# paulmillr/noble-curves

Hardware: AMD Instinct MI355X
Metric: secp256k1_scalar_mults_per_sec (higher is better)
Workload: dtype u32

## Files before the change

### noble-curves_amd/csrc/ec_sw.hpp

```cpp
#pragma once
#include "fp2.hpp"

namespace ncg {

template <class A, class B, class C, class D>
NCG_DI auto f_mulsub(const A& a, const B& b, const C& c, const D& d) -> decltype(a * b - c * d) {
  return a * b - c * d;
}


template <class F>
struct Affine {
  F x, y;
  NCG_DI bool is_inf() const { return x.is_zero() && y.is_zero(); }
};

template <class F>
struct Jac {
  F X, Y, Z;
  static NCG_DI Jac inf() { return {F::one(), F::one(), F::zero()}; }
  NCG_DI bool is_inf() const { return Z.is_zero(); }
};

template <class F>
// ... 43 lines not shown
  auto S2 = qy * p.Z * Z1Z1;
  auto H = U2 - p.X;
  auto R = S2 - p.Y;
  if (f_eqz(H)) {
    if (f_eqz(R)) return jac_dbl(p);
    return Jac<F>::inf();
  }
  auto HH = f_sqr(H);
  auto HHH = H * HH;
  auto V = p.X * HH;
  auto X3 = f_sqr(R) - HHH - f_dbl(V);
  auto Y3 = R * (V - X3) - p.Y * HHH;
  auto Z3 = p.Z * H;
  return {X3, Y3, Z3};
}
template <class F, class FX, class FY>
NCG_DI Jac<F> jac_madd_q(const Jac<F>& p, const FX& qx, const FY& qy) {
  if (qx.is_zero() && qy.is_zero()) return p;
  if (p.is_inf()) return {qx, qy, F::one()};
  return jac_madd_xy(p, qx, qy);
}
template <class F>
NCG_DI Jac<F> jac_madd(const Jac<F>& p, const Affine<F>& q) {
  return jac_madd_q(p, q.x, q.y);
}

template <class F>
NCG_DI Jac<F> jac_add(const Jac<F>& p, const Jac<F>& q) {
  if (q.is_inf()) return p;
  if (p.is_inf()) return q;
  auto Z1Z1 = f_sqr(p.Z);
  auto Z2Z2 = f_sqr(q.Z);
  auto U1 = p.X * Z2Z2;
  auto U2 = q.X * Z1Z1;
  auto S1 = p.Y * q.Z * Z2Z2;
  auto S2 = q.Y * p.Z * Z1Z1;
  auto H = U2 - U1;
  auto R = S2 - S1;
  if (f_eqz(H)) {
    if (f_eqz(R)) return jac_dbl(p);
    return Jac<F>::inf();
  }
  auto HH = f_sqr(H);
  auto HHH = H * HH;
  auto V = U1 * HH;
  auto X3 = f_sqr(R) - HHH - f_dbl(V);
  auto Y3 = R * (V - X3) - S1 * HHH;
  auto Z3 = p.Z * q.Z * H;
  return {X3, Y3, Z3};
}

template <class F, class ZI>
NCG_DI Affine<F> jac_to_affine(const Jac<F>& p, const ZI& zinv) {
  if (p.is_inf()) return {F::zero(), F::zero()};
  auto zi2 = f_sqr(zinv);
  return {p.X * zi2, p.Y * zi2 * zinv};
}

template <class PR, int B>
NCG_DI Jac<Fe9<PR, B>> jac_dbl(const Jac<Fe9<PR, B>>& p) {
  auto A = f_sqr(p.X);
  auto Bq = f_sqr(p.Y);
  auto C8 = f_dbl(f_sqr(f_dbl(Bq)));
  auto D = fe9_norm(f_dbl(f_dbl(p.X * Bq)));
  auto E = fe9_norm(A + A + A);
  auto X3 = f_sqr(E) - f_dbl(D);
  auto Y3 = E * (D - X3) - C8;
  auto Z3 = f_dbl(p.Y * p.Z);
  return {X3, Y3, Z3};
}

template <class PR, int B, int BX, int BY>
NCG_DI Jac<Fe9<PR, B>> jac_madd_xy(const Jac<Fe9<PR, B>>& p, const Fe9<PR, BX>& qx, const Fe9<PR, BY>& qy) {
  using F = Fe9<PR, B>;
  auto Z1Z1 = f_sqr(p.Z);
  auto U2 = qx * Z1Z1;
  auto S2 = qy * (p.Z * Z1Z1);
  auto Hw = U2 - p.X;
  auto Rw = S2 - p.Y;
  if (f_eqz(Hw)) {
    if (f_eqz(Rw)) return jac_dbl(p);
    return Jac<F>::inf();
  }
  auto H = fe9_norm(Hw);
  auto R = fe9_norm(Rw);
  auto HH = f_sqr(H);
  auto HHH = H * HH;
  auto V = p.X * HH;
  auto X3 = fe9_norm(f_sqr(R) - HHH - f_dbl(V));
  auto Y3 = R * (V - X3) - p.Y * HHH;
  auto Z3 = p.Z * H;
  return {X3, Y3, Z3};
}
template <class PR, int B>
NCG_DI Jac<Fe9<PR, B>> jac_add(const Jac<Fe9<PR, B>>& p, const Jac<Fe9<PR, B>>& q) {
  using F = Fe9<PR, B>;
  if (q.is_inf()) return p;
  if (p.is_inf()) return q;
  auto Z1Z1 = f_sqr(p.Z);
  auto Z2Z2 = f_sqr(q.Z);
  auto U1 = p.X * Z2Z2;
  auto U2 = q.X * Z1Z1;
  auto S1 = p.Y * (q.Z * Z2Z2);
  auto S2 = q.Y * (p.Z * Z1Z1);
  auto Hw = U2 - U1;
  auto Rw = S2 - S1;
  if (f_eqz(Hw)) {
    if (f_eqz(Rw)) return jac_dbl(p);
    return Jac<F>::inf();
  }
  auto H = fe9_norm(Hw);
  auto R = fe9_norm(Rw);
  auto HH = f_sqr(H);
  auto HHH = H * HH;
  auto V = U1 * HH;
  auto X3 = fe9_norm(f_sqr(R) - HHH - f_dbl(V));
  auto Y3 = R * (V - X3) - S1 * HHH;
  auto Z3 = (p.Z * q.Z) * H;
  return {X3, Y3, Z3};
}

template <class PR, int B>
NCG_DI Jac<Fe9<PR, B>> jac_dbl_neg(const Jac<Fe9<PR, B>>& p) {
  auto A = f_sqr(p.X);
  auto S = f_sqr(p.Y);
  auto T = p.X * S;
  auto L = f_half(fe9_norm(A + A + A));
  auto X3 = f_sqr_add(L, f_neg_lin2(T));
  auto W = f_mul_sqr(L, X3 - T, S);
  auto Z3 = p.Y * p.Z;
  return {X3, W, Z3};
}

template <class PR, int B, int BX, int BY>
NCG_DI Jac<Fe9<PR, B>> jac_madd_neg(const Jac<Fe9<PR, B>>& p, const Fe9<PR, BX>& qx, const Fe9<PR, BY>& qy) {
  using F = Fe9<PR, B>;
  if (qx.is_zero() && qy.is_zero()) return {p.X, f_neg(p.Y), p.Z};
  if (p.is_inf()) return {qx, f_neg(qy), F::one()};
  auto Z1Z1 = f_sqr(p.Z);
  auto Z1Z1Z1 = p.Z * Z1Z1;
  auto H = f_mul_add(qx, Z1Z1, f_neg_lin(p.X));
  auto R = f_mul_add(qy, Z1Z1Z1, f_neg_lin(p.Y));
  if (f_eqz(H)) {
    if (f_eqz(R)) return jac_dbl_neg(p);
    return Jac<F>::inf();
  }
  auto HH = f_sqr(H);
  auto HHH = H * HH;
  auto V = p.X * HH;
  auto X3 = f_sqr_add(R, f_neg_lin(HHH, V));
  auto W = f_mul_mul(R, X3 - V, p.Y, HHH);
  auto Z3 = p.Z * H;
  return {X3, W, Z3};
}

template <class F>
NCG_DI Xyzz<F> xyzz_from_affine(const Affine<F>& p) {
  if (p.is_inf()) return Xyzz<F>::inf();
  return {p.x, p.y, F::one(), F::one()};
}

template <class F>
NCG_DI Xyzz<F> xyzz_mdbl(const Affine<F>& p) {
  auto U = f_dbl(p.y);
  auto V = f_sqr(U);
  auto W = U * V;
  auto S = p.x * V;
  auto xx = f_sqr(p.x);
  auto M = f_dbl(xx) + xx;
  auto X3 = f_sqr(M) - f_dbl(S);
  auto Y3 = f_mulsub(M, S - X3, W, p.y);
  return {X3, Y3, V, W};
}

template <class F>
NCG_DI Xyzz<F> xyzz_dbl(const Xyzz<F>& p) {
  if (p.is_inf()) return p;
  auto U = f_dbl(p.Y);
  auto V = f_sqr(U);
  auto W = U * V;
  auto S = p.X * V;
  auto xx = f_sqr(p.X);
  auto M = f_dbl(xx) + xx;
  auto X3 = f_sqr(M) - f_dbl(S);
  auto Y3 = f_mulsub(M, S - X3, W, p.Y);
  return {X3, Y3, V * p.ZZ, W * p.ZZZ};
}

template <class F>
NCG_DI Xyzz<F> xyzz_madd(const Xyzz<F>& p, const Affine<F>& q_in, bool neg = false) {
  if (q_in.is_inf()) return p;
  Affine<F> q = q_in;
  if (neg) q.y = f_neg(q.y);
  if (p.is_inf()) return {q.x, q.y, F::one(), F::one()};
  auto U2 = q.x * p.ZZ;
  auto S2 = q.y * p.ZZZ;
  auto Pq = U2 - p.X;
  auto R = S2 - p.Y;
  if (f_eqz(Pq)) {
    if (f_eqz(R)) return xyzz_mdbl(q);
    return Xyzz<F>::inf();
  }
  auto PP = f_sqr(Pq);
  auto PPP = Pq * PP;
  auto Q = p.X * PP;
  auto X3 = f_sqr(R) - PPP - f_dbl(Q);
  auto Y3 = f_mulsub(R, Q - X3, p.Y, PPP);
  return {X3, Y3, p.ZZ * PP, p.ZZZ * PPP};
}

template <class F>
NCG_DI Xyzz<F> xyzz_add(const Xyzz<F>& p, const Xyzz<F>& q) {
  if (q.is_inf()) return p;
  if (p.is_inf()) return q;
  auto U1 = p.X * q.ZZ;
  auto U2 = q.X * p.ZZ;
  auto S1 = p.Y * q.ZZZ;
  auto S2 = q.Y * p.ZZZ;
  auto Pq = U2 - U1;
  auto R = S2 - S1;
  if (f_eqz(Pq)) {
    if (f_eqz(R)) return xyzz_dbl(p);
    return Xyzz<F>::inf();
  }
  auto PP = f_sqr(Pq);
  auto PPP = Pq * PP;
  auto Q = U1 * PP;
  auto X3 = f_sqr(R) - PPP - f_dbl(Q);
  auto Y3 = f_mulsub(R, Q - X3, S1, PPP);
  return {X3, Y3, p.ZZ * q.ZZ * PP, p.ZZZ * q.ZZZ * PPP};
}

template <class PR, int B>
NCG_DI Xyzz<Fe9<PR, B>> xyzz_mdbl(const Affine<Fe9<PR, B>>& p) {
  auto U = f_dbl(p.y);
  auto V = f_sqr(U);
  auto W = U * V;
  auto S = p.x * V;
  auto xx = f_sqr(p.x);
  auto M = fe9_norm(xx + xx + xx);
  auto X3 = fe9_norm(f_sqr(M) - f_dbl(S));
  auto Y3 = M * (S - X3) - W * p.y;
  return {X3, Y3, V, W};
}
template <class PR, int B>
NCG_DI Xyzz<Fe9<PR, B>> xyzz_dbl(const Xyzz<Fe9<PR, B>>& p) {
  if (p.is_inf()) return p;
  auto U = f_dbl(p.Y);
  auto V = f_sqr(U);
  auto W = U * V;
  auto S = p.X * V;
  auto xx = f_sqr(p.X);
  auto M = fe9_norm(xx + xx + xx);
  auto X3 = fe9_norm(f_sqr(M) - f_dbl(S));
  auto Y3 = M * (S - X3) - W * p.Y;
  return {X3, Y3, V * p.ZZ, W * p.ZZZ};
}
template <class PR, int B>
NCG_DI Xyzz<Fe9<PR, B>> xyzz_madd(const Xyzz<Fe9<PR, B>>& p, const Affine<Fe9<PR, B>>& q_in, bool neg = false) {
  using F = Fe9<PR, B>;
  if (q_in.is_inf()) return p;
  const Fe9<PR, B + 1> qy = neg ? f_neg(q_in.y) : Fe9<PR, B + 1>(q_in.y);
  if (p.is_inf()) return {q_in.x, qy, F::one(), F::one()};
  auto U2 = q_in.x * p.ZZ;
  auto S2 = qy * p.ZZZ;
  auto Pw = U2 - p.X;
  auto Rw = S2 - p.Y;
  if (f_eqz(Pw)) {
    if (f_eqz(Rw)) return xyzz_mdbl(Affine<F>{q_in.x, qy});
    return Xyzz<F>::inf();
  }
  auto Pq = fe9_norm(Pw);
  auto R = fe9_norm(Rw);
  auto PP = f_sqr(Pq);
  auto PPP = Pq * PP;
  auto Q = p.X * PP;
  auto X3 = fe9_norm(f_sqr(R) - PPP - f_dbl(Q));
  auto Y3 = R * (Q - X3) - p.Y * PPP;
  return {X3, Y3, p.ZZ * PP, p.ZZZ * PPP};
}
template <class PR, int B>
NCG_DI Xyzz<Fe9<PR, B>> xyzz_add(const Xyzz<Fe9<PR, B>>& p, const Xyzz<Fe9<PR, B>>& q) {
  using F = Fe9<PR, B>;
  if (q.is_inf()) return p;
  if (p.is_inf()) return q;
  auto U1 = p.X * q.ZZ;
  auto U2 = q.X * p.ZZ;
  auto S1 = p.Y * q.ZZZ;
  auto S2 = q.Y * p.ZZZ;
  auto Pw = U2 - U1;
  auto Rw = S2 - S1;
  if (f_eqz(Pw)) {
    if (f_eqz(Rw)) return xyzz_dbl(p);
    return Xyzz<F>::inf();
  }
  auto Pq = fe9_norm(Pw);
  auto R = fe9_norm(Rw);
  auto PP = f_sqr(Pq);
  auto PPP = Pq * PP;
  auto Q = U1 * PP;
  auto X3 = fe9_norm(f_sqr(R) - PPP - f_dbl(Q));
  auto Y3 = R * (Q - X3) - S1 * PPP;
  return {X3, Y3, (p.ZZ * q.ZZ) * PP, (p.ZZZ * q.ZZZ) * PPP};
}

}
// ... 1 lines not shown
```

### noble-curves_amd/csrc/fe9.hpp

```cpp
#pragma once
#include <type_traits>

#include "fp.hpp"
#include "fe9_asm_gen.hpp"
#include "fe9m.hpp"

namespace ncg {

constexpr uint32_t FE9_MASK = (1u << 29) - 1u;

template <class PR, class = void> struct Fe9IsMont : std::false_type {};
template <class PR> struct Fe9IsMont<PR, std::void_t<decltype(PR::MONT)>> : std::integral_constant<bool, PR::MONT> {};

template <class PR>
struct Fe9Raw {
  uint32_t v[9];
};

NCG_DI void fe9_mac(uint64_t& acc, uint32_t a, uint32_t b) {
#ifdef __HIP_DEVICE_COMPILE__
  asm("v_mad_u64_u32 %0, vcc, %1, %2, %0" : "+v"(acc) : "v"(a), "v"(b) : "vcc");
#else
  acc += (uint64_t)a * b;
#endif
// ... 224 lines not shown
  static NCG_DI Fe9 zero() {
    Fe9 r;
#pragma unroll
    for (int i = 0; i < 9; i++) r.v[i] = 0;
    return r;
  }
  static NCG_DI Fe9 one() {
    Fe9 r = zero();
    if constexpr (Fe9IsMont<PR>::value) {
#pragma unroll
      for (int i = 0; i < 9; i++) r.v[i] = PR::ONE[i];
    } else {
      r.v[0] = 1;
    }
    return r;
  }
  template <class ARR>
  static NCG_DI Fe9 from_limbs(const ARR& a) {
    Fe9 r;
#pragma unroll
    for (int i = 0; i < 9; i++) r.v[i] = a[i];
    return r;
  }
  NCG_DI bool is_zero() const {
    uint32_t o = 0;
#pragma unroll
    for (int i = 0; i < 9; i++) o |= v[i];
    return o == 0;
  }
};

template <class PR, int B>
NCG_DI Fe9<PR, 1> fe9_norm(const Fe9<PR, B>& a) {
  if constexpr (B == 1) return a;
  else return Fe9<PR, 1>(a);
}

template <class PR, int A, int B>
NCG_DI Fe9<PR, A + B> operator+(const Fe9<PR, A>& a, const Fe9<PR, B>& b) {
  Fe9<PR, A + B> r;
#pragma unroll
  for (int i = 0; i < 9; i++) r.v[i] = a.v[i] + b.v[i];
  return r;
}
template <class PR, int A, int B>
NCG_DI Fe9<PR, A + B + 1> operator-(const Fe9<PR, A>& a, const Fe9<PR, B>& b) {
  Fe9<PR, A + B + 1> r;
#pragma unroll
  for (int i = 0; i < 9; i++) {
#ifdef __HIP_DEVICE_COMPILE__
    asm("v_sad_u32 %0, %1, %2, %3" : "=v"(r.v[i]) : "s"(PR::BIAS[B][i]), "v"(b.v[i]), "v"(a.v[i]));
#else
    r.v[i] = a.v[i] + (PR::BIAS[B][i] - b.v[i]);
#endif
  }
  return r;
}
template <class PR, int A>
NCG_DI Fe9<PR, A + 1> f_neg(const Fe9<PR, A>& a) {
  Fe9<PR, A + 1> r;
  const bool z = a.is_zero();
#pragma unroll
  for (int i = 0; i < 9; i++) r.v[i] = z ? 0u : PR::BIAS[A][i] - a.v[i];
  return r;
}
template <class PR, int A>
NCG_DI Fe9<PR, 2 * A> f_dbl(const Fe9<PR, A>& a) {
  Fe9<PR, 2 * A> r;
#pragma unroll
  for (int i = 0; i < 9; i++) r.v[i] = a.v[i] << 1;
  return r;
}

template <class PR, int A, int B>
NCG_DI Fe9<PR, 1> operator*(const Fe9<PR, A>& a, const Fe9<PR, B>& b) {
  if constexpr (A * B > 7) {
    if constexpr (A >= B) return fe9_norm(a) * b;
    else return a * fe9_norm(b);
  } else {
    Fe9Raw<PR> x, y;
#pragma unroll
    for (int i = 0; i < 9; i++) {
      x.v[i] = a.v[i];
      y.v[i] = b.v[i];
    }
    const Fe9Raw<PR> z = fe9_mul_raw<PR>(x, y);
    Fe9<PR, 1> r;
#pragma unroll
    for (int i = 0; i < 9; i++) r.v[i] = z.v[i];
    return r;
  }
}
template <class PR, int A>
NCG_DI Fe9<PR, 1> f_sqr(const Fe9<PR, A>& a) {
  if constexpr (A > 2) {
    return f_sqr(fe9_norm(a));
  } else {
    Fe9Raw<PR> x;
#pragma unroll
    for (int i = 0; i < 9; i++) x.v[i] = a.v[i];
    const Fe9Raw<PR> z = fe9_sqr_raw<PR>(x);
    Fe9<PR, 1> r;
#pragma unroll
    for (int i = 0; i < 9; i++) r.v[i] = z.v[i];
    return r;
  }
}

template <class PR, int KIND, int A, int B, int C, int D>
NCG_DI Fe9<PR, 1> fe9_fused(const Fe9<PR, A>& a, const Fe9<PR, B>& b, const Fe9<PR, C>& f, const Fe9<PR, D>& g) {
  Fe9<PR, 1> r;
  fe9_fused_limbs<PR, KIND>(r.v, a.v, b.v, f.v, g.v);
  return r;
}
template <class PR, int A, int B, int C, int D>
NCG_DI Fe9<PR, 1> f_mul_mul(const Fe9<PR, A>& a, const Fe9<PR, B>& b, const Fe9<PR, C>& c, const Fe9<PR, D>& d) {
  static_assert(A * B + C * D <= 7, "fused a*b + c*d: the two products overflow the 64-bit columns");
  return fe9_fused<PR, FE9_MM>(a, b, c, d);
}
template <class PR, int A, int B, int C>
NCG_DI Fe9<PR, 1> f_mul_sqr(const Fe9<PR, A>& a, const Fe9<PR, B>& b, const Fe9<PR, C>& c) {
  static_assert(C <= 2 && A * B + C * C <= 7, "fused a*b + c^2: the two sources overflow the 64-bit columns");
  return fe9_fused<PR, FE9_MS>(a, b, c, f_dbl(c));
}
template <class PR, int A, int B, int S>
NCG_DI Fe9<PR, 1> f_mul_add(const Fe9<PR, A>& a, const Fe9<PR, B>& b, const Fe9<PR, S>& s) {
  static_assert(A * B <= 7, "fused a*b + s: the product overflows the 64-bit columns");
  return fe9_fused<PR, FE9_MA>(a, b, s, s);
}
template <class PR, int A, int S>
NCG_DI Fe9<PR, 1> f_sqr_add(const Fe9<PR, A>& a, const Fe9<PR, S>& s) {
  static_assert(A <= 2, "fused a^2 + s: the square overflows the 64-bit columns");
  return fe9_fused<PR, FE9_SA>(a, f_dbl(a), s, s);
}
template <class PR, int S1, int S2>
NCG_DI Fe9<PR, S1 + 2 * S2 + 1> f_neg_lin(const Fe9<PR, S1>& s1, const Fe9<PR, S2>& s2) {
  Fe9<PR, S1 + 2 * S2 + 1> r;
#pragma unroll
  for (int i = 0; i < 9; i++) r.v[i] = PR::BIAS[S1 + 2 * S2][i] - (s1.v[i] + (s2.v[i] << 1));
  return r;
}
template <class PR, int S1>
NCG_DI Fe9<PR, S1 + 1> f_neg_lin(const Fe9<PR, S1>& s1) {
  Fe9<PR, S1 + 1> r;
#pragma unroll
  for (int i = 0; i < 9; i++) r.v[i] = PR::BIAS[S1][i] - s1.v[i];
  return r;
}
template <class PR, int S2>
NCG_DI Fe9<PR, 2 * S2 + 1> f_neg_lin2(const Fe9<PR, S2>& s2) {
  Fe9<PR, 2 * S2 + 1> r;
#pragma unroll
  for (int i = 0; i < 9; i++) r.v[i] = PR::BIAS[2 * S2][i] - (s2.v[i] << 1);
  return r;
}
template <class PR>
NCG_DI Fe9<PR, 2> f_half(const Fe9<PR, 1>& a) {
  const uint32_t m = 0u - (a.v[0] & 1u);
  uint32_t t[9];
#pragma unroll
  for (int i = 0; i < 9; i++) t[i] = a.v[i] + (PR::P[i] & m);
  Fe9<PR, 2> r;
#pragma unroll
  for (int i = 0; i < 8; i++) r.v[i] = (t[i] >> 1) + ((t[i + 1] & 1u) << 28);
  r.v[8] = t[8] >> 1;
  return r;
}

template <class PR>
NCG_DI Fe9<PR, 1> fe9_sqr_n(Fe9<PR, 1> a, int n) {
  for (int i = 0; i < n; i++) a = f_sqr(a);
  return a;
}

template <class PR, int A>
NCG_DI void fe9_canon_limbs_sf(uint32_t (&o)[9], const Fe9<PR, A>& a);
template <class PR, int A>
NCG_DI void fe9_canon_limbs(uint32_t (&o)[9], const Fe9<PR, A>& a) {
  if constexpr (Fe9IsMont<PR>::value) {
    uint32_t t[9];
    fe9m_reduce(t, a.v);
    fe9m_cond_sub(o, t);
  } else {
    fe9_canon_limbs_sf<PR, A>(o, a);
  }
}
template <class PR, int A>
NCG_DI void fe9_canon_limbs_sf(uint32_t (&o)[9], const Fe9<PR, A>& a) {
  uint64_t cy = 0;
  uint32_t t[9];
#pragma unroll
  for (int i = 0; i < 9; i++) {
    cy += a.v[i];
    t[i] = (uint32_t)cy & FE9_MASK;
    cy >>= 29;
  }
#pragma unroll
  for (int pass = 0; pass < 2; pass++) {
    uint64_t e = (uint64_t)(uint32_t)cy * PR::C0 + t[0];
    t[0] = (uint32_t)e & FE9_MASK;
    e >>= 29;
    e += (uint64_t)(uint32_t)cy * PR::C1 + t[1];
    t[1] = (uint32_t)e & FE9_MASK;
    e >>= 29;
#pragma unroll
    for (int i = 2; i < 9; i++) {
      e += t[i];
      t[i] = (uint32_t)e & FE9_MASK;
      e >>= 29;
    }
    cy = e;
  }
  constexpr int PBITS = (PR::P[8] >> 23) ? 256 : 255;
  constexpr int TOPB = PBITS - 232;
  constexpr uint32_t CSM = (uint32_t)((1ull << 29) - PR::P[0]);
  constexpr uint32_t CS1 = FE9_MASK - PR::P[1];
#pragma unroll
  for (int pass = 0; pass < 2; pass++) {
    const uint32_t q = t[8] >> TOPB;
    t[8] &= (1u << TOPB) - 1u;
    uint64_t e = (uint64_t)q * CSM + t[0];
    t[0] = (uint32_t)e & FE9_MASK;
    e >>= 29;
    e += (uint64_t)q * CS1 + t[1];
    t[1] = (uint32_t)e & FE9_MASK;
    e >>= 29;
#pragma unroll
    for (int i = 2; i < 9; i++) {
      e += t[i];
      t[i] = (uint32_t)e & FE9_MASK;
      e >>= 29;
    }
  }
  uint32_t s[9];
  int32_t bw = 0;
#pragma unroll
  for (int i = 0; i < 9; i++) {
    int32_t dd = (int32_t)t[i] - (int32_t)PR::P[i] + bw;
    s[i] = (uint32_t)dd & FE9_MASK;
    bw = dd >> 29;
  }
  const bool ge = bw == 0;
#pragma unroll
  for (int i = 0; i < 9; i++) o[i] = ge ? s[i] : t[i];
}

template <class PR, class... T>
__host__ __device__ __noinline__ bool fe9_eqz_slow(T... limbs) {
  Fe9<PR, 7> a;
  const uint32_t v[9] = {limbs...};
#pragma unroll
  for (int i = 0; i < 9; i++) a.v[i] = v[i];
  uint32_t c[9];
  fe9_canon_limbs<PR, 7>(c, a);
  uint32_t o = 0;
#pragma unroll
  for (int i = 0; i < 9; i++) o |= c[i];
  return o == 0;
}
template <class PR, int A>
NCG_DI bool f_eqz(const Fe9<PR, A>& a) {
  const uint32_t j = (a.v[0] * PR::PINV) & FE9_MASK;
  if (j >= (uint32_t)(PR::JMAX * A)) return false;
  return fe9_eqz_slow<PR>(a.v[0], a.v[1], a.v[2], a.v[3], a.v[4], a.v[5], a.v[6], a.v[7], a.v[8]);
}
template <class PR, int A, int B>
NCG_DI bool f_eq(const Fe9<PR, A>& a, const Fe9<PR, B>& b) {
  return f_eqz(a - b);
}

template <class PR>
NCG_DI Fe9<PR, 1> fe9_from_wire(const uint32_t* __restrict__ p) {
  if constexpr (Fe9IsMont<PR>::value) {
    Fe9<PR, 1> r;
    fe9m_from_wire(r.v, p);
    return r;
  }
  uint32_t w[10];
#pragma unroll
  for (int i = 0; i < 8; i++) w[i] = p[i];
  w[8] = 0;
  w[9] = 0;
  Fe9<PR, 1> r;
#pragma unroll
  for (int i = 0; i < 9; i++) {
    const int bit = 29 * i, limb = bit >> 5, sh = bit & 31;
    const uint64_t two = ((uint64_t)w[limb + 1] << 32) | w[limb];
    r.v[i] = (uint32_t)(two >> sh) & FE9_MASK;
  }
  return r;
}
template <class PR, int A>
NCG_DI void fe9_to_wire(uint32_t* __restrict__ p, const Fe9<PR, A>& a) {
  if constexpr (Fe9IsMont<PR>::value) {
    uint32_t c[9];
    fe9m_canon_plain(c, fe9_norm(a).v);
    fe9m_words_from_limbs(p, c);
    return;
  }
  uint32_t l[11];
  uint32_t c[9];
  fe9_canon_limbs<PR, A>(c, a);
#pragma unroll
  for (int i = 0; i < 9; i++) l[i] = c[i];
  l[9] = 0;
  l[10] = 0;
// ... 77 lines not shown
```

### noble-curves_amd/csrc/hosttest.hip

```cpp
#include <vector>

#include "../../include/ncg.h"
#include "mulvar.hpp"
#include "ed25519.hip"
#include "decode.hip"
#include "ntt.hip"
#include "poly.hip"
#include "h2c.hip"
#include "endo.hpp"
#include "ecdsa.hip"
#include "msm_shard.hpp"
#include "msm_endo.hip"
#include "msm_schedule.hpp"
#include "fe9m_check.hpp"
#include "group_check.hpp"
#include "x25519.hip"
#include "ristretto.hip"

using namespace ncg;

template <class C, int W>
static void ht_mul_var_t(const uint32_t* pts, const uint32_t* scalars, uint32_t* out, uint8_t* out_inf, int n) {
  constexpr int FW = MulVarCfg<C, W>::FW, WW = MulVarCfg<C, W>::WW;
  std::vector<uint32_t> tab(MulVarCfg<C, W>::TS * 2 * FW);
// ... 192 lines not shown
  }
  Fe9<PR, 1> o;
  if constexpr (A * B + C * D <= 7) {
    if (op == 0) o = f_mul_mul(x, y, z, w);
  }
  if constexpr (C <= 2 && A * B + C * C <= 7) {
    if (op == 1) o = f_mul_sqr(x, y, z);
  }
  if constexpr (A * B <= 7) {
    if (op == 2) o = f_mul_add(x, y, z);
  }
  if constexpr (A <= 2) {
    if (op == 3) o = f_sqr_add(x, z);
  }
  if constexpr (A == 1) {
    if (op == 4) {
      const Fe9<PR, 2> h = f_half(x);
      for (int i = 0; i < 9; i++) r[i] = h.v[i];
      return;
    }
  }
  for (int i = 0; i < 9; i++) r[i] = o.v[i];
}
template <class PR>
static int ht_fe9_fused_t(int op, int variant, const uint32_t* a, const uint32_t* b, const uint32_t* c, const uint32_t* d, uint32_t* r) {
  switch (variant) {
    case 1111: ht_fe9_fused_ab<PR, 1, 1, 1, 1>(op, a, b, c, d, r); return 0;
    case 1322: ht_fe9_fused_ab<PR, 1, 3, 2, 2>(op, a, b, c, d, r); return 0;
    case 3211: ht_fe9_fused_ab<PR, 3, 2, 1, 1>(op, a, b, c, d, r); return 0;
    case 2311: ht_fe9_fused_ab<PR, 2, 3, 1, 1>(op, a, b, c, d, r); return 0;
    case 1123: ht_fe9_fused_ab<PR, 1, 1, 2, 3>(op, a, b, c, d, r); return 0;
    case 3121: ht_fe9_fused_ab<PR, 3, 1, 2, 1>(op, a, b, c, d, r); return 0;
    case 1327: ht_fe9_fused_ab<PR, 1, 3, 2, 7>(op, a, b, c, d, r); return 0;
    case 7171: ht_fe9_fused_ab<PR, 7, 1, 7, 1>(op, a, b, c, d, r); return 0;
    case 1771: ht_fe9_fused_ab<PR, 1, 7, 7, 1>(op, a, b, c, d, r); return 0;
    case 2171: ht_fe9_fused_ab<PR, 2, 1, 7, 1>(op, a, b, c, d, r); return 0;
    default: return -1;
  }
}

template <class F>
static int fr29_op_host(int op, const uint32_t* a, const uint32_t* b, uint32_t* r) {
  Fr29 x, y, z;
  for (int i = 0; i < 9; i++) {
    x.v[i] = a[i];
    y.v[i] = b ? b[i] : 0;
    z.v[i] = 0;
  }
  fr29_overflows() = 0;
  switch (op) {
    case 0: z = fr29_mont<F>(x, y); break;
    case 1: z = fr29_add(x, y); break;
    case 2: z = fr29_sub<F>(x, y); break;
    case 3: z = fr29_weak(x); break;
    case 4: z = fr29_reduce256<F>(x); break;
    case 5: z = fr29_cond_sub<F>(x); break;
    case 8: z = fr29_fold255<F>(x); break;
    case 6: {
      uint32_t w[8];
      for (int i = 0; i < 8; i++) w[i] = a[i];
      z = fr29_from_words(w);
      break;
    }
    case 7: {
      uint32_t w[8];
      fr29_to_words(w, x);
      for (int i = 0; i < 8; i++) z.v[i] = w[i];
      z.v[8] = 0;
      break;
    }
    default: return -1;
  }
  for (int i = 0; i < 9; i++) r[i] = z.v[i];
  return fr29_overflows();
}

template <class PR, int A>
static void ht_fe9_inv_batch_t(int which, const uint32_t* a, uint32_t* out, uint32_t* raw, int n) {
  for (int k = 0; k < n; k++) {
    Fe9<PR, A> x;
    for (int i = 0; i < 9; i++) x.v[i] = a[(size_t)k * 9 + i];
    const Fe9<PR, 1> z = which ? f_inv_fermat(x) : f_inv(x);
    fe9_to_wire(out + (size_t)k * 8, z);
    if (raw)
      for (int i = 0; i < 9; i++) raw[(size_t)k * 9 + i] = z.v[i];
  }
}

extern "C" {

int ht_fe9_op(int field, int op, int variant, const uint32_t* a, const uint32_t* b, uint32_t* r) {
  if (field == 0) return ht_fe9_t<Fe9SecpPR>(op, variant, a, b, r);
  if (field == 1) return ht_fe9_t<Fe9EdPR>(op, variant, a, b, r);
  return -1;
}

int ht_fe9_inv_batch(int field, int A, int which, const uint32_t* a, uint32_t* out, uint32_t* raw, int n) {
  if (field < 0 || field > 1 || (A != 1 && A != 2 && A != 7)) return -1;
#define CALL(PR) (A == 1 ? ht_fe9_inv_batch_t<PR, 1>(which, a, out, raw, n) : A == 2 ? ht_fe9_inv_batch_t<PR, 2>(which, a, out, raw, n) : ht_fe9_inv_batch_t<PR, 7>(which, a, out, raw, n))
  if (field == 0) CALL(Fe9SecpPR);
  else CALL(Fe9EdPR);
#undef CALL
  return 0;
}

int ht_mul_var(int curve, const uint32_t* pts, const uint32_t* scalars, uint32_t* out, uint8_t* out_inf, int n) {
  switch (curve) {
    case CURVE_SECP256K1: ht_mul_var_t<CurveSecp, 4>(pts, scalars, out, out_inf, n); return 0;
    case CURVE_BLS12_381_G1: ht_mul_var_t<CurveG1, 3>(pts, scalars, out, out_inf, n); return 0;
    case 12: ht_mul_var_t<CurveG1E, 4>(pts, scalars, out, out_inf, n); return 0;
    case 14: ht_mul_var_t<CurveSecpI, 4>(pts, scalars, out, out_inf, n); return 0;
    case CURVE_BLS12_381_G2: ht_mul_var_t<CurveG2, 3>(pts, scalars, out, out_inf, n); return 0;
    case CURVE_BN254_G1: ht_mul_var_t<CurveBn254, 4>(pts, scalars, out, out_inf, n); return 0;
  }
  return -1;
}

int ht_field_op(int field, int op, const uint32_t* a, const uint32_t* b, uint32_t* r) {
  switch (field) {
    case 0: ht_field_t<ParamsSecpP>(op, a, b, r); return 0;
    case 1: ht_field_t<ParamsEdP>(op, a, b, r); return 0;
    case 2: ht_field_t<ParamsBlsP>(op, a, b, r); return 0;
  }
  return -1;
}

int ht_fe9_fused(int field, int op, int variant, const uint32_t* a, const uint32_t* b, const uint32_t* c, const uint32_t* d,
                 uint32_t* r) {
  if (field == 0) return ht_fe9_fused_t<Fe9SecpPR>(op, variant, a, b, c, d, r);
  if (field == 1) return ht_fe9_fused_t<Fe9EdPR>(op, variant, a, b, c, d, r);
  return -1;
}

int ht_jac_neg(int op, const uint32_t* p, const uint32_t* qx, const uint32_t* qy, uint32_t* out) {
  Jac<FeSecp> P;
  Fe9<Fe9SecpPR, 2> x;
  Fe9<Fe9SecpPR, 3> y;
  for (int i = 0; i < 9; i++) {
    P.X.v[i] = p[i];
    P.Y.v[i] = p[9 + i];
    P.Z.v[i] = p[18 + i];
    x.v[i] = qx[i];
    y.v[i] = qy[i];
  }
  Jac<FeSecp> R;
  if (op == 0) R = jac_dbl_neg(P);
  else if (op == 1) R = jac_madd_neg(P, x, y);
  else return -1;
  for (int i = 0; i < 9; i++) {
    out[i] = R.X.v[i];
    out[9 + i] = R.Y.v[i];
    out[18 + i] = R.Z.v[i];
  }
  return 0;
}

int ht_glv_split_odd(const uint32_t* k, uint32_t* out) {
  uint32_t kk[8];
  for (int i = 0; i < 8; i++) kk[i] = k[i];
  GlvSplit s = secp_glv_split(kk);
  secp_glv_make_odd(s);
  for (int i = 0; i < 5; i++) {
    out[i] = s.k1[i];
    out[5 + i] = s.k2[i];
  }
  out[10] = s.k1neg;
  out[11] = s.k2neg;
  return 0;
}

int ht_glv_split_k1_odd(const uint32_t* k, uint32_t* out) {
  uint32_t kk[8];
  for (int i = 0; i < 8; i++) kk[i] = k[i];
  GlvSplit s = secp_glv_split(kk);
  secp_glv_make_k1_odd(s);
  for (int i = 0; i < 5; i++) {
    out[i] = s.k1[i];
    out[5 + i] = s.k2[i];
  }
  out[10] = s.k1neg;
  out[11] = s.k2neg;
  return 0;
}

int ht_glv_split(const uint32_t* k, uint32_t* out) {
  uint32_t kk[8];
  for (int i = 0; i < 8; i++) kk[i] = k[i];
  GlvSplit s = secp_glv_split(kk);
  for (int i = 0; i < 5; i++) {
    out[i] = s.k1[i];
    out[5 + i] = s.k2[i];
  }
  out[10] = s.k1neg;
  out[11] = s.k2neg;
  return 0;
}

int ht_ed25519_mul_var(const uint32_t* pts, const uint32_t* scalars, uint32_t* out, uint8_t* out_inf, int n) {
  for (int i = 0; i < n; i++) ed25519_mul_var_host(pts + (size_t)i * 16, scalars + (size_t)i * 8, out + (size_t)i * 16, out_inf + i);
  return 0;
}

int ht_x25519(const uint32_t* scalars, const uint32_t* u, int flags, uint32_t* out, uint8_t* ok, int n) {
  if (flags & ~1) return -1;
  x25519_host(scalars, u, flags & 1, out, ok, n);
  return 0;
}
int ht_x25519_base(const uint32_t* scalars, uint32_t* out, uint8_t* ok, int n) {
  x25519_base_host(scalars, out, ok, n);
  return 0;
}
int ht_ed25519_to_montgomery(const uint32_t* pk, uint32_t* out, uint8_t* ok, int n) {
  ed25519_to_montgomery_host(pk, out, ok, n);
  return 0;
}
int ht_x25519_op(int op, int variant, const uint32_t* a, const uint32_t* b, uint32_t* out) { return x25519_check_host(op, variant, a, b, out); }

int ht_ristretto_decode(const uint32_t* enc, uint32_t* out_affine, uint8_t* ok, int n) {
  ristretto_decode_host(enc, out_affine, ok, 0, n);
  return 0;
}
int ht_ristretto_encode(const uint32_t* affine, uint32_t* out, int n) {
  ristretto_encode_host(affine, out, n);
  return 0;
}
int ht_ristretto_encode_proj(const uint32_t* proj_wire, uint32_t* out, int n) {
  ristretto_encode_proj_host(proj_wire, out, n);
  return 0;
}
int ht_ristretto_equals(const uint32_t* a, const uint32_t* b, uint8_t* eq, int n) {
  ristretto_equals_host(a, b, eq, n);
  return 0;
}
int ht_ristretto_from_uniform(const uint32_t* bytes64, uint32_t* out, uint32_t* out_affine, int n) {
  ristretto_from_uniform_host(bytes64, out, out_affine, n);
  return 0;
}
int ht_ristretto_mul(const uint32_t* enc, const uint32_t* scalars, int flags, uint32_t* out, uint8_t* ok, int n) {
  if (flags & ~1) return -1;
  ristretto_mul_host(enc, scalars, flags & 1, out, ok, n);
  return 0;
}
int ht_ristretto_op(int op, const uint32_t* a, const uint32_t* b, uint32_t* out) { return ristretto_check_host(op, a, b, out); }
int ht_ristretto_consts(uint32_t* out32) {
  fe9_to_wire(out32, RistrettoConsts::sqrt_ad_minus_one());
  fe9_to_wire(out32 + 8, RistrettoConsts::invsqrt_a_minus_d());
  fe9_to_wire(out32 + 16, RistrettoConsts::one_minus_d_sq());
  fe9_to_wire(out32 + 24, RistrettoConsts::d_minus_one_sq());
  return 0;
}

int ht_fp2_sqrt(const uint32_t* in, uint32_t* out) {
  Fe29x2<2> a{fe29_from_wire(in), fe29_from_wire(in + 12)}, r;
  bool ok = fe29x2_sqrt(a, r);
  fe29_to_wire(out, r.c0);
  fe29_to_wire(out + 12, r.c1);
  return ok ? 1 : 0;
}

int ht_decode_points(int curve, const uint8_t* in, int flags, uint32_t* out, uint8_t* ok, uint8_t* inf, int n) {
  decode_points_host(curve, in, flags, out, ok, inf, n);
  return 0;
}

int ht_encode_points(int curve, const uint32_t* in, uint8_t* out, uint8_t* ok, int n) {
  encode_points_host(curve, in, out, ok, n);
  return 0;
}

int ht_map_to_curve(int curve, const uint32_t* u, int count, uint32_t* out, uint8_t* inf, int n) {
  map_to_curve_host(curve, u, count, out, inf, n);
  return 0;
}

int ht_ntt(int n, const uint32_t* omega, const uint32_t* in, uint32_t* out, int flags) {
  return ntt_host(NCG_FIELD_BLS12_381_FR, n, omega, in, out, flags);
}
int ht_ntt_small_passes(int n, const uint32_t* omega, const uint32_t* in, uint32_t* out, int flags, int t0max, int tmax) {
  if (t0max < 1 || tmax < 1 || 1 + (n - (n < t0max ? n : t0max) + tmax - 1) / tmax > 8) return -1;
  return ntt_host(NCG_FIELD_BLS12_381_FR, n, omega, in, out, flags, t0max, tmax);
}
int ht_ntt_field(int field, int n, const uint32_t* omega, const uint32_t* in, uint32_t* out, int flags, int t0max, int tmax) {
  if (field != NCG_FIELD_BLS12_381_FR && field != NCG_FIELD_BN254_FR) return -1;
  if (t0max == 0 && tmax == 0) return ntt_host(field, n, omega, in, out, flags);
  if (t0max < 1 || tmax < 1 || 1 + (n - (n < t0max ? n : t0max) + tmax - 1) / tmax > 8) return -1;
  return ntt_host(field, n, omega, in, out, flags, t0max, tmax);
}
int ht_fr29_op(int op, const uint32_t* a, const uint32_t* b, uint32_t* r) {
  if (op < 0 || op > 7) return -1;
  return fr29_op_host<Fr29Bls>(op, a, b, r);
}
int ht_fr29_field_op(int variant, int op, const uint32_t* a, const uint32_t* b, uint32_t* r) {
  if (variant == 0) return fr29_op_host<Fr29Bls>(op, a, b, r);
  if (variant == 1) return fr29_op_host<Fr29Bn>(op, a, b, r);
  return -1;
}
int ht_fe9m_op(int op, int variant, const uint32_t* a, const uint32_t* b, uint32_t* r) {
  fe9m_overflows() = 0;
  if (fe9m_check(op, variant, a, b, r) != 0) return -1;
  return fe9m_overflows();
}
int ht_group_op(int field, int op, const uint32_t* a, const uint32_t* b, uint32_t* out) {
  if (op < 0 || op > 3) return -1;
  switch (field) {
    case 10: group_check_op<CurveSecp>(op, a, b, out); return 0;
    case 11: group_check_op<CurveEd>(op, a, b, out); return 0;
// ... 254 lines not shown
```

### noble-curves_amd/csrc/mulvar.hpp

```cpp
#pragma once
#include <type_traits>

#include "curves.hpp"
#include "scalar.hpp"

namespace ncg {

template <class F>
NCG_DI void coz_addu(Affine<F>& D, Affine<F>& T, F& zr, bool& degenerate) {
  auto dx = D.x - T.x;
  degenerate = degenerate || f_eqz(dx);
  auto C = f_sqr(dx);
  auto W1 = D.x * C;
  auto W2 = T.x * C;
  auto dy = D.y - T.y;
  auto A1 = D.y * (W1 - W2);
  auto X3 = f_sqr(dy) - W1 - W2;
  auto Y3 = dy * (W1 - X3) - A1;
  zr = dx * F::one();
  D = {W1, A1};
  T = {X3, Y3};
}
template <class PR, int B>
NCG_DI void coz_addu(Affine<Fe9<PR, B>>& D, Affine<Fe9<PR, B>>& T, Fe9<PR, B>& zr, bool& degenerate) {
  auto dxw = D.x - T.x;
  degenerate = degenerate || f_eqz(dxw);
  auto dx = fe9_norm(dxw);
  auto dy = fe9_norm(D.y - T.y);
  auto C = f_sqr(dx);
  auto W1 = D.x * C;
  auto W2 = T.x * C;
  auto A1 = D.y * (W1 - W2);
  auto X3 = fe9_norm(f_sqr(dy) - W1 - W2);
  auto Y3 = dy * (W1 - X3) - A1;
  zr = dx;
  D = {W1, A1};
  T = {X3, Y3};
}

template <class C>
NCG_DI Jac<typename C::F> mul_var_slow(const uint32_t* __restrict__ pt_wire, const uint32_t* __restrict__ k_wire) {
  using F = typename C::F;
  const Affine<F> P = load_affine_wire<F>(pt_wire);
  Jac<F> R = Jac<F>::inf();
  for (int w = 7; w >= 0; w--) {
    const uint32_t word = k_wire[w];
    for (int bit = 31; bit >= 0; bit--) {
      R = jac_dbl(R);
      if ((word >> bit) & 1u) R = jac_madd(R, P);
    }
  }
  return R;
}

template <class C, class = void> struct OddGlvHalves { static constexpr bool value = false; };
template <class C> struct OddGlvHalves<C, std::void_t<decltype(C::ODD_HALVES)>> { static constexpr bool value = C::GLV && C::ODD_HALVES; };
template <class C, class = void> struct OddK1Half { static constexpr bool value = false; };
template <class C> struct OddK1Half<C, std::void_t<decltype(C::K1_ODD)>> { static constexpr bool value = C::GLV && C::K1_ODD; };
template <class C, class = void> struct FusedLadder { static constexpr bool value = false; };
template <class C> struct FusedLadder<C, std::void_t<decltype(C::FUSED_LADDER)>> { static constexpr bool value = C::FUSED_LADDER; };

template <class C, int W>
struct MulVarCfg {
  using F = typename C::F;
  static constexpr int FW = FieldIO<F>::WORDS;
  static constexpr int TW = FieldIO<F>::LANE_WORDS;
  static constexpr int WW = FieldWire<F>::WORDS;
  static constexpr int TS = 1 << (W - 1);
  static constexpr int KBITS = OddK1Half<C>::value ? 128 : C::GLV ? 129 : 257;
  static constexpr int M = (KBITS + W - 1) / W;
  static constexpr int NL = (KBITS + 31) / 32;
  static constexpr int LDS_WORDS = TS * 2 * TW * 64;
};

template <class C, int W, bool JAC_OUT = false, bool ZR_IN_TAB = false, class TABPTR>
NCG_DI void mul_var_lane(const uint32_t* __restrict__ pt_wire, const uint32_t* __restrict__ k_wire,
                         uint32_t* __restrict__ out_wire, uint8_t* __restrict__ out_inf, bool active,
                         TABPTR tab, const int stride) {
  using Cfg = MulVarCfg<C, W>;
  using F = typename C::F;
  constexpr int FW = Cfg::FW, TW = Cfg::TW, TS = Cfg::TS, M = Cfg::M, NL = Cfg::NL;

  Affine<F> P = load_affine_wire<F>(pt_wire);
  uint32_t k[8];
#pragma unroll
  for (int i = 0; i < 8; i++) k[i] = k_wire[i];
  const bool trivial_zero = P.is_inf() || mp_is_zero<8>(k);

  F Zg;
  bool degenerate = false;
  {
    Jac<F> D = jac_dbl(Jac<F>{P.x, P.y, F::one()});
    auto dz2 = f_sqr(D.Z);
    auto dz3 = dz2 * D.Z;
    Affine<F> Dc{D.X, D.Y};
    Affine<F> T{P.x * dz2, P.y * dz3};
    F zr[ZR_IN_TAB ? 1 : TS];
    auto zr_put = [&](int j, const F& v) {
      if constexpr (ZR_IN_TAB) FieldIO<F>::store_strided(tab + (TS * 2 * TW + j * TW) * stride, stride, v);
      else zr[j] = v;
    };
    auto zr_get = [&](int j) -> F {
      if constexpr (ZR_IN_TAB) return FieldIO<F>::load_strided(tab + (TS * 2 * TW + j * TW) * stride, stride);
      else return zr[j];
    };
    FieldIO<F>::store_strided(tab, stride, T.x);
    FieldIO<F>::store_strided(tab + TW * stride, stride, T.y);
#pragma unroll(ZR_IN_TAB ? 1 : TS)
    for (int j = 1; j < TS; j++) {
      F zj;
      coz_addu(Dc, T, zj, degenerate);
      zr_put(j, zj);
      FieldIO<F>::store_strided(tab + (j * 2 * TW) * stride, stride, T.x);
      FieldIO<F>::store_strided(tab + (j * 2 * TW + TW) * stride, stride, T.y);
    }
    F s = F::one();
#pragma unroll(ZR_IN_TAB ? 1 : TS)
    for (int j = TS - 2; j >= 0; j--) {
      if (j == TS - 2) s = zr_get(j + 1);
      else s = s * zr_get(j + 1);
      auto s2 = f_sqr(s);
      auto s3 = s2 * s;
      F x = FieldIO<F>::load_strided(tab + (j * 2 * TW) * stride, stride);
      F y = FieldIO<F>::load_strided(tab + (j * 2 * TW + TW) * stride, stride);
      FieldIO<F>::store_strided(tab + (j * 2 * TW) * stride, stride, x * s2);
      FieldIO<F>::store_strided(tab + (j * 2 * TW + TW) * stride, stride, y * s3);
    }
    Zg = D.Z * s;
  }

  SignedOddWindows<NL, W, M> w1, w2;
  bool neg1 = false, neg2 = false;
  constexpr bool ODD = OddGlvHalves<C>::value;
  constexpr bool K1ODD = OddK1Half<C>::value;
  if constexpr (C::GLV) {
    GlvSplit gs = C::glv_split(k);
    if constexpr (ODD) secp_glv_make_odd(gs);
    if constexpr (K1ODD) secp_glv_make_k1_odd(gs);
    w1.template init<5>(gs.k1);
    w2.template init<5>(gs.k2);
    neg1 = gs.k1neg;
    neg2 = gs.k2neg;
  } else {
    w1.template init<8>(k);
  }
  const auto beta = C::beta();

  constexpr bool FUSED = FusedLadder<C>::value;
  bool sg = false;
  auto dbl = [&](const Jac<F>& r) -> Jac<F> {
    if constexpr (FUSED) {
      sg = !sg;
      return jac_dbl_neg(r);
    } else {
      return jac_dbl(r);
    }
  };
  auto madd = [&](const Jac<F>& r, const auto& qx, const F& qy, bool ng) -> Jac<F> {
    if constexpr (FUSED) {
      const bool s = sg;
      sg = !sg;
      return jac_madd_neg(r, qx, f_cneg(qy, ng != s));
    } else {
      return jac_madd_q(r, qx, f_cneg(qy, ng));
    }
  };
  Jac<F> R = Jac<F>::inf();
  for (int i = 0; i < M; i++) {
    if (i > 0) {
#pragma unroll(NCG_MUL_INLINE ? 1 : W)
      for (int d = 0; d < W; d++) R = dbl(R);
    }
    if constexpr (NCG_MUL_INLINE && C::GLV) {
#pragma unroll 1
      for (int e = 0; e < 2; e++) {
        const int d = e == 0 ? w1.pop() : w2.pop();
        const bool ng = e == 0 ? neg1 : neg2;
        const int idx = ((d < 0 ? -d : d) - 1) >> 1;
        F qx = FieldIO<F>::load_strided(tab + (idx * 2 * TW) * stride, stride);
        const F qy = FieldIO<F>::load_strided(tab + (idx * 2 * TW + TW) * stride, stride);
        if (e == 1) qx = qx * beta;
        R = madd(R, qx, qy, (d < 0) != ng);
      }
    } else {
      {
        int d1 = w1.pop();
        int e = ((d1 < 0 ? -d1 : d1) - 1) >> 1;
        const F qx = FieldIO<F>::load_strided(tab + (e * 2 * TW) * stride, stride);
        const F qy = FieldIO<F>::load_strided(tab + (e * 2 * TW + TW) * stride, stride);
        R = madd(R, qx, qy, (d1 < 0) != neg1);
      }
      if constexpr (C::GLV) {
        int d2 = w2.pop();
        int e = ((d2 < 0 ? -d2 : d2) - 1) >> 1;
        const auto qx = FieldIO<F>::load_strided(tab + (e * 2 * TW) * stride, stride) * beta;
        const F qy = FieldIO<F>::load_strided(tab + (e * 2 * TW + TW) * stride, stride);
        R = madd(R, qx, qy, (d2 < 0) != neg2);
      }
    }
  }
  if constexpr (!ODD) {
    const F qx = FieldIO<F>::load_strided(tab, stride);
    const F qy = FieldIO<F>::load_strided(tab + TW * stride, stride);
    if constexpr (!K1ODD) {
      if (w1.was_even) R = madd(R, qx, qy, !neg1);
    }
    if constexpr (C::GLV) {
      if (w2.was_even) R = madd(R, qx * beta, qy, !neg2);
    }
  }
  if constexpr (FUSED) {
    if (sg) R.Y = f_neg(R.Y);
  }
  const bool ladder_inf = R.is_inf();
  R.Z = R.Z * Zg;
  if (ladder_inf) R = Jac<F>::inf();
  if (degenerate) R = mul_var_slow<C>(pt_wire, k_wire);
  bool inf = trivial_zero || R.is_inf();
  if constexpr (JAC_OUT) {
    if (inf) R = Jac<F>::inf();
    if (active) {
      FieldIO<F>::store(out_wire, R.X);
      FieldIO<F>::store(out_wire + FW, R.Y);
      FieldIO<F>::store(out_wire + 2 * FW, R.Z);
    }
    return;
  }
  Affine<F> A = jac_to_affine(R, f_inv(R.Z));
  if (inf) A = {F::zero(), F::zero()};
  if (active) {
    store_affine_wire<F>(out_wire, A);
    *out_inf = inf ? 1 : 0;
  }
}

template <class C, int K, bool PRE_LDS = false>
__global__ void __launch_bounds__(PRE_LDS ? 64 : 256) k_jac_batch_affine(const uint32_t* __restrict__ jac,
                                                                         uint32_t* __restrict__ out_wire,
                                                                         uint8_t* __restrict__ out_inf, int n) {
  using F = typename C::F;
  constexpr int FW = FieldIO<F>::WORDS, WW = FieldWire<F>::WORDS, TW = FieldIO<F>::LANE_WORDS;
  extern __shared__ __attribute__((aligned(16))) uint32_t pre_lds[];
  const int t = (blockIdx.x * blockDim.x + threadIdx.x) >> LaneShift<C>::value;
  const int i0 = t * K;
  if (i0 >= n) return;
  F pre[PRE_LDS ? 1 : K];
  auto pre_put = [&](int j, const F& v) {
    if constexpr (PRE_LDS) FieldIO<F>::store_strided(pre_lds + threadIdx.x + (size_t)j * TW * 64, 64, v);
    else pre[j] = v;
  };
  auto pre_get = [&](int j) -> F {
    if constexpr (PRE_LDS) return FieldIO<F>::load_strided(pre_lds + threadIdx.x + (size_t)j * TW * 64, 64);
    else return pre[j];
  };
  F acc = F::one();
#pragma unroll
  for (int j = 0; j < K; j++) {
    pre_put(j, acc);
    if (i0 + j < n) {
      F z = FieldIO<F>::load(jac + ((size_t)(i0 + j) * 3 + 2) * FW);
      if (!z.is_zero()) acc = acc * z;
    }
  }
  F inv = f_inv(acc);
#pragma unroll
  for (int j = K - 1; j >= 0; j--) {
    if (i0 + j < n) {
      const uint32_t* p = jac + (size_t)(i0 + j) * 3 * FW;
      F z = FieldIO<F>::load(p + 2 * FW);
      const bool inf = z.is_zero();
      Affine<F> A{F::zero(), F::zero()};
      if (!inf) {
        F zi = inv * pre_get(j);
        inv = inv * z;
        auto zi2 = f_sqr(zi);
        A = {FieldIO<F>::load(p) * zi2, FieldIO<F>::load(p + FW) * zi2 * zi};
      }
      store_affine_wire<F>(out_wire + (size_t)(i0 + j) * 2 * WW, A);
      out_inf[i0 + j] = inf ? 1 : 0;
    }
  }
}

template <class F, int K>
__global__ void __launch_bounds__(256) k_proj_batch_affine(const uint32_t* __restrict__ proj_wire,
                                                           uint32_t* __restrict__ out_wire,
                                                           uint8_t* __restrict__ out_inf, int n) {
  constexpr int WW = FieldWire<F>::WORDS;
  const int t = blockIdx.x * blockDim.x + threadIdx.x;
  const int i0 = t * K;
  if (i0 >= n) return;
  F pre[K];
  F acc = F::one();
#pragma unroll
  for (int j = 0; j < K; j++) {
    pre[j] = acc;
    if (i0 + j < n) {
      F z = FieldWire<F>::load(proj_wire + ((size_t)(i0 + j) * 3 + 2) * WW);
      if (!f_eqz(z)) acc = acc * z;
    }
  }
  F inv = f_inv(acc);
#pragma unroll
  for (int j = K - 1; j >= 0; j--) {
    if (i0 + j < n) {
      const uint32_t* p = proj_wire + (size_t)(i0 + j) * 3 * WW;
      F z = FieldWire<F>::load(p + 2 * WW);
      const bool inf = f_eqz(z);
      F x = F::zero(), y = F::zero();
      if (!inf) {
        F zi = inv * pre[j];
        inv = inv * z;
        x = FieldWire<F>::load(p) * zi;
        y = FieldWire<F>::load(p + WW) * zi;
      }
      FieldWire<F>::store(out_wire + (size_t)(i0 + j) * 2 * WW, x);
      FieldWire<F>::store(out_wire + (size_t)(i0 + j) * 2 * WW + WW, y);
      out_inf[i0 + j] = inf ? 1 : 0;
    }
  }
}

template <class C, int W, int MINW, bool JAC_OUT>
__global__ void __launch_bounds__(64, MINW)
k_mul_var_gtab(const uint32_t* __restrict__ pts, const uint32_t* __restrict__ scalars, uint32_t* __restrict__ out,
               uint8_t* __restrict__ out_inf, uint32_t* __restrict__ gtab, int n) {
  using Cfg = MulVarCfg<C, W>;
  constexpr int WW = Cfg::WW;
  constexpr int OUTW = JAC_OUT ? 3 * Cfg::FW : 2 * WW;
  const int lane_idx = blockIdx.x * 64 + threadIdx.x;
  const int idx = lane_idx >> LaneShift<C>::value;
  const bool active = idx < n;
  const int src = active ? idx : n - 1;
  mul_var_lane<C, W, JAC_OUT, true>(pts + (size_t)src * 2 * WW, scalars + (size_t)src * 8, out + (size_t)src * OUTW,
                                    out_inf + src, active, gtab + (size_t)lane_idx * (Cfg::TS * 3 * Cfg::TW), 1);
}

template <class C, int W, int MINW, bool JAC_OUT>
__global__ void __launch_bounds__(64, MINW)
k_mul_var(const uint32_t* __restrict__ pts, const uint32_t* __restrict__ scalars,
          uint32_t* __restrict__ out, uint8_t* __restrict__ out_inf, int n) {
  constexpr int WW = MulVarCfg<C, W>::WW;
  constexpr int OUTW = JAC_OUT ? 3 * MulVarCfg<C, W>::FW : 2 * WW;
  extern __shared__ __attribute__((aligned(16))) uint32_t lds[];
  const int lane = threadIdx.x;
  const int idx = (blockIdx.x * 64 + lane) >> LaneShift<C>::value;
  const bool active = idx < n;
  const int src = active ? idx : n - 1;
  mul_var_lane<C, W, JAC_OUT>(pts + (size_t)src * 2 * WW, scalars + (size_t)src * 8, out + (size_t)src * OUTW,
                              out_inf + src, active, lds + lane, 64);
}

template <class C, int W>
inline size_t gtab_words_per_item() { return (size_t)MulVarCfg<C, W>::TS * 3 * MulVarCfg<C, W>::TW; }
inline size_t pad64(size_t n) { return (n + 63) / 64 * 64; }

template <class C, int W, int MINW, int K = 8>
inline hipError_t launch_mul_var_gtab(const uint32_t* pts, const uint32_t* scalars, uint32_t* out, uint8_t* out_inf,
                                      int n, uint32_t* jac_tmp, hipStream_t st) {
  if (n <= 0) return hipSuccess;
  using Cfg = MulVarCfg<C, W>;
  constexpr int LS = LaneShift<C>::value;
  uint32_t* gtab = jac_tmp + pad64(n) * 3 * Cfg::FW;
  const unsigned blocks = (unsigned)((((size_t)n << LS) + 63) / 64);
  hipLaunchKernelGGL((k_mul_var_gtab<C, W, MINW, true>), dim3(blocks), dim3(64), 0, st, pts, scalars, jac_tmp, out_inf,
// ... 9 lines not shown
```

Baseline: 136.8 million.

## Use exception-free mixed add in fused ladder and seed with affine first add

The fused GLV ladder now uses a mixed-add variant that drops the infinity and H==0 branch checks and instead records a degenerate flag, which sends the rare cases to the existing slow fallback path. The first window is handled as a direct affine+affine addition of the two table points, avoiding doublings of infinity and a general madd. Negation uses a lazy (unreduced) conditional negate. This removes divergent branches and some field operations per step, at the cost of relying on the slow-path fallback being correct for every degenerate input.

Measured after the change: 139.1 million, median of 6. 1.02x the previous value.

```diff
diff --git a/noble-curves_amd/csrc/ec_sw.hpp b/noble-curves_amd/csrc/ec_sw.hpp
--- a/noble-curves_amd/csrc/ec_sw.hpp
+++ b/noble-curves_amd/csrc/ec_sw.hpp
@@ -219,6 +219,36 @@
   auto W = f_mul_mul(R, X3 - V, p.Y, HHH);
   auto Z3 = p.Z * H;
   return {X3, W, Z3};
+}
+
+template <class PR, int B, int BX, int BY>
+NCG_DI Jac<Fe9<PR, B>> jac_madd_neg_nx(const Jac<Fe9<PR, B>>& p, const Fe9<PR, BX>& qx, const Fe9<PR, BY>& qy, bool& degenerate) {
+  auto Z1Z1 = f_sqr(p.Z);
+  auto Z1Z1Z1 = p.Z * Z1Z1;
+  auto H = f_mul_add(qx, Z1Z1, f_neg_lin(p.X));
+  auto R = f_mul_add(qy, Z1Z1Z1, f_neg_lin(p.Y));
+  degenerate |= f_eqz(H);
+  auto HH = f_sqr(H);
+  auto HHH = H * HH;
+  auto V = p.X * HH;
+  auto X3 = f_sqr_add(R, f_neg_lin(HHH, V));
+  auto W = f_mul_mul(R, X3 - V, p.Y, HHH);
+  auto Z3 = p.Z * H;
+  return {X3, W, Z3};
+}
+
+template <class PR, int B, int BY>
+NCG_DI Jac<Fe9<PR, B>> aff_add_neg_nx(const Fe9<PR, B>& x1, const Fe9<PR, BY>& y1, const Fe9<PR, B>& x2, const Fe9<PR, 1>& b,
+                                      const Fe9<PR, BY>& y2, bool& degenerate) {
+  auto H = f_mul_add(x2, b, f_neg_lin(x1));
+  auto R = fe9_norm(y2 - y1);
+  degenerate |= f_eqz(H);
+  auto HH = f_sqr(H);
+  auto HHH = H * HH;
+  auto V = x1 * HH;
+  auto X3 = f_sqr_add(R, f_neg_lin(HHH, V));
+  auto W = f_mul_mul(R, X3 - V, y1, HHH);
+  return {X3, W, H};
 }
 
 template <class F>
diff --git a/noble-curves_amd/csrc/fe9.hpp b/noble-curves_amd/csrc/fe9.hpp
--- a/noble-curves_amd/csrc/fe9.hpp
+++ b/noble-curves_amd/csrc/fe9.hpp
@@ -400,6 +400,13 @@
   Fe9<PR, 2 * S2 + 1> r;
 #pragma unroll
   for (int i = 0; i < 9; i++) r.v[i] = PR::BIAS[2 * S2][i] - (s2.v[i] << 1);
+  return r;
+}
+template <class PR, int A>
+NCG_DI Fe9<PR, A + 1> f_cneg_lin(const Fe9<PR, A>& a, bool c) {
+  Fe9<PR, A + 1> r;
+#pragma unroll
+  for (int i = 0; i < 9; i++) r.v[i] = c ? PR::BIAS[A][i] - a.v[i] : a.v[i];
   return r;
 }
 template <class PR>
diff --git a/noble-curves_amd/csrc/hosttest.hip b/noble-curves_amd/csrc/hosttest.hip
--- a/noble-curves_amd/csrc/hosttest.hip
+++ b/noble-curves_amd/csrc/hosttest.hip
@@ -368,6 +368,31 @@
     out[9 + i] = R.Y.v[i];
     out[18 + i] = R.Z.v[i];
   }
+  return 0;
+}
+
+int ht_jac_neg_nx(int op, const uint32_t* p, const uint32_t* qx, const uint32_t* qy, uint32_t* out) {
+  Jac<FeSecp> P;
+  Fe9<Fe9SecpPR, 2> x;
+  Fe9<Fe9SecpPR, 3> y;
+  for (int i = 0; i < 9; i++) {
+    P.X.v[i] = p[i];
+    P.Y.v[i] = p[9 + i];
+    P.Z.v[i] = p[18 + i];
+    x.v[i] = qx[i];
+    y.v[i] = qy[i];
+  }
+  Jac<FeSecp> R;
+  bool degenerate = false;
+  if (op == 0) R = jac_madd_neg_nx(P, x, y, degenerate);
+  else if (op == 1) R = aff_add_neg_nx(P.X, Fe9<Fe9SecpPR, 3>(P.Y), x, CurveSecpI::beta(), y, degenerate);
+  else return -1;
+  for (int i = 0; i < 9; i++) {
+    out[i] = R.X.v[i];
+    out[9 + i] = R.Y.v[i];
+    out[18 + i] = R.Z.v[i];
+  }
+  out[27] = degenerate ? 1u : 0u;
   return 0;
 }
 
diff --git a/noble-curves_amd/csrc/mulvar.hpp b/noble-curves_amd/csrc/mulvar.hpp
--- a/noble-curves_amd/csrc/mulvar.hpp
+++ b/noble-curves_amd/csrc/mulvar.hpp
@@ -147,6 +147,7 @@
   const auto beta = C::beta();
 
   constexpr bool FUSED = FusedLadder<C>::value;
+  static_assert(!FUSED || (C::GLV && OddK1Half<C>::value), "the fused ladder is the GLV ladder with k1 odd");
   bool sg = false;
   auto dbl = [&](const Jac<F>& r) -> Jac<F> {
     if constexpr (FUSED) {
@@ -160,18 +161,27 @@
     if constexpr (FUSED) {
       const bool s = sg;
       sg = !sg;
-      return jac_madd_neg(r, qx, f_cneg(qy, ng != s));
+      return jac_madd_neg_nx(r, qx, f_cneg_lin(qy, ng != s), degenerate);
     } else {
       return jac_madd_q(r, qx, f_cneg(qy, ng));
     }
   };
   Jac<F> R = Jac<F>::inf();
-  for (int i = 0; i < M; i++) {
-    if (i > 0) {
+  if constexpr (FUSED) {
+    const int d1 = w1.pop(), d2 = w2.pop();
+    const int e1 = ((d1 < 0 ? -d1 : d1) - 1) >> 1, e2 = ((d2 < 0 ? -d2 : d2) - 1) >> 1;
+    const F x1 = FieldIO<F>::load_strided(tab + (e1 * 2 * TW) * stride, stride);
+    const F y1 = FieldIO<F>::load_strided(tab + (e1 * 2 * TW + TW) * stride, stride);
+    const F x2 = FieldIO<F>::load_strided(tab + (e2 * 2 * TW) * stride, stride);
+    const F y2 = FieldIO<F>::load_strided(tab + (e2 * 2 * TW + TW) * stride, stride);
+    R = aff_add_neg_nx(x1, f_cneg_lin(y1, (d1 < 0) == neg1), x2, beta, f_cneg_lin(y2, (d2 < 0) == neg2), degenerate);
+  }
+  for (int i = FUSED ? 1 : 0; i < M; i++) {
+    if (FUSED || i > 0) {
 #pragma unroll(NCG_MUL_INLINE ? 1 : W)
       for (int d = 0; d < W; d++) R = dbl(R);
     }
-    if constexpr (NCG_MUL_INLINE && C::GLV) {
+    if constexpr (NCG_MUL_INLINE && C::GLV && !FUSED) {
 #pragma unroll 1
       for (int e = 0; e < 2; e++) {
         const int d = e == 0 ? w1.pop() : w2.pop();
@@ -211,6 +221,7 @@
   }
   if constexpr (FUSED) {
     if (sg) R.Y = f_neg(R.Y);
+    degenerate = degenerate && !trivial_zero;
   }
   const bool ladder_inf = R.is_inf();
   R.Z = R.Z * Zg;
```
